# ChainSafe/halo2-verifier

Measured on NVIDIA B200. Metric: verified proofs/sec (BN254 SHPLONK, batch 4096), higher is better.
Workload: dtype u32x8 (256-bit Montgomery integers)

## Files before the change

__graft_entry__.py:

```python
import importlib.util
import os
import subprocess
import sys

ROOT = os.path.dirname(os.path.abspath(__file__))
PKG_DIR = os.path.join(ROOT, "halo2-verifier_b200")
CSRC = os.path.join(PKG_DIR, "csrc")
LIB = os.path.join(PKG_DIR, "libh2v_b200.so")
HOSTLIB = os.path.join(ROOT, "tests", "hostlib")
ORACLE = os.path.join(ROOT, "oracle")

NVCC_FLAGS = [
    "-gencode", "arch=compute_100a,code=sm_100a", "-lineinfo", "-O3", "-std=c++17",
    "-Xcompiler", "-fPIC", "-shared", "-I", os.path.join(ROOT, "include"), "-I", CSRC,
]


def load_package():
    name = "halo2_verifier_b200"
    if name in sys.modules:
        return sys.modules[name]
    spec = importlib.util.spec_from_file_location(name, os.path.join(PKG_DIR, "__init__.py"),
                                                  submodule_search_locations=[PKG_DIR])
    mod = importlib.util.module_from_spec(spec)
    sys.modules[name] = mod
    spec.loader.exec_module(mod)
    return mod


def _newer(target, sources):
    if not os.path.exists(target):
        return True
    t = os.path.getmtime(target)
    return any(os.path.getmtime(s) > t for s in sources)


def _run(cmd):
    print("+", " ".join(cmd), flush=True)
    subprocess.run(cmd, check=True)


def build(force=False):
    headers = [os.path.join(CSRC, f) for f in os.listdir(CSRC)] + [os.path.join(ROOT, "include", "h2v.h")]
    if force or _newer(LIB, headers):
        nvcc = os.environ.get("NVCC", "/usr/local/cuda/bin/nvcc")
        _run([nvcc] + NVCC_FLAGS + [os.path.join(CSRC, "kernels.cu"), os.path.join(CSRC, "plan_build.cpp"), "-o", LIB])
    for name, srcs in (("libprim.so", ["prim_harness.cpp"]), ("libstage.so", ["stage_harness.cpp", os.path.join(CSRC, "plan_build.cpp")]),
                       ("libmix.so", ["mix_harness.cpp"]), ("libacc.so", ["acc_harness.cpp"]),
                       ("libagg.so", ["agg_harness.cpp"])):
        out = os.path.join(HOSTLIB, name)
        full = [s if os.path.isabs(s) else os.path.join(HOSTLIB, s) for s in srcs]
        if force or _newer(out, headers + full):
            cmd = ["g++", "-O2", "-std=c++17", "-shared", "-fPIC", "-I", CSRC]
            for s in full:
                cmd += ["-x", "c++", s]
            _run(cmd + ["-o", out])
    mk = os.path.join(ORACLE, "Makefile")
    if os.path.exists(mk):
        _run(["make", "-s", "-C", ORACLE])
    load_package()


def smoke():
    import random

    sys.path.insert(0, ORACLE)
    import bn254 as bn
    import prover_sim as sim
    import verifier as orc

    pkg = load_package()
    rng = random.Random(11)
    k, s = 8, sim.FIXTURE_SRS_SECRET
    params = sim.make_params(k, s)
    vk, dl = sim.make_vk("vm", k)
    n = 8
    instances = [sim.random_instances(vk, rng, 10) for _ in range(n)]
    proofs = [sim.simulate_proof(params, vk, dl, s, inst, rng) for inst in instances]
    proofs[3], _ = sim.corrupt(proofs[3], vk, "eval_flip", rng)
    rs = [rng.randrange(1, bn.R) for _ in range(n)]
    bv = pkg.BatchVerifier(pkg.ParamsKZG.from_bytes(params.to_bytes()), pkg.VerifyingKey.from_bytes(vk.to_bytes(1)), device=0)
    res = bv.verify_batch(proofs, [i[0] for i in instances], rlc_scalars=rs, want_challenges=True, want_batch_accum=True)
    want = [orc.verify_proof(params, vk, inst, p) for inst, p in zip(instances, proofs)]
    assert res.status == [w.status for w in want], (res.status, [w.status for w in want])
    C = bv.n_challenges
    for j, w in enumerate(want):
        got = [int.from_bytes(res.challenges[32 * (j * C + c): 32 * (j * C + c + 1)], "little") for c in range(C)]
        assert got == w.challenges, f"challenge mismatch on proof {j}"
    L, Rr, _ok = orc.accumulate(params, want, rs)
    enc = lambda p: bytes(64) if p is None else p[0].to_bytes(32, "little") + p[1].to_bytes(32, "little")
    assert res.batch_accum == enc(L) + enc(Rr), "folded accumulator mismatch"
    print("smoke ok: statuses", res.status, "launches", bv.launch_count(), "timings(ms)", bv.timings())
    bv.close()


if __name__ == "__main__":
    build(force="--force" in sys.argv)
    if "--smoke" in sys.argv:
        smoke()
```

halo2-verifier_b200/csrc/kernels.cu:

```cuda
#include <cuda_runtime.h>
#include <nvtx3/nvToolsExt.h>
#include <errno.h>
#include <stdio.h>
#include <string.h>
#include <sys/random.h>
#include <time.h>
#include <unistd.h>

#include <algorithm>
#include <cmath>
#include <string>
#include <vector>

#include "h2v.h"
#include "plan_build.h"
#include "stages.cuh"
#include "tower.cuh"
#include "timeline.cuh"
#include "pairing_cta.cuh"
#include "exchange.cuh"
#include "transcript_quad.cuh"
#include "glv.cuh"
#include "mix.cuh"
#include "acc.cuh"
#include "agg.cuh"

using namespace h2v;

#ifndef H2V_TRANSCRIPT_MINB
#define H2V_TRANSCRIPT_MINB 1
#endif
#ifndef H2V_SCALAR_MINB
#define H2V_SCALAR_MINB 1
#endif

__device__ __forceinline__ void pdl_prologue() {
  asm volatile("griddepcontrol.wait;" ::: "memory");
  asm volatile("griddepcontrol.launch_dependents;" ::: "memory");
}

__global__ void k_init(PlanView pv, u32 n, const u64* inst_off, const u32* ncols, const u32* col_len, u32* status, u32* bad) {
  pdl_prologue();
  const u32 j = blockIdx.x * blockDim.x + threadIdx.x;
  if (j >= n) return;
  const PlanHeader& hd = pv.h();
  bad[j] = H2V_NO_BAD_ITEM;
  const u64 tot = inst_off[j + 1] - inst_off[j];
  u32 st = ST_OK;
  if (ncols && ncols[j] != hd.n_inst_cols) {
    st = ST_INVALID_INSTANCES;
  } else if (col_len) {
    u64 s = 0;
    for (u32 c = 0; c < hd.n_inst_cols; c++) s += col_len[(size_t)j * hd.n_inst_cols + c];
    if (s != tot) st = ST_INVALID_INSTANCES;
  } else if (hd.n_inst_cols == 0 ? tot != 0 : (tot % hd.n_inst_cols) != 0) {
    st = ST_INVALID_INSTANCES;
  }
  status[j] = st;
}

__global__ void __launch_bounds__(128) k_decompress(PlanView pv, u32 n, const u8* proofs, const u64* proof_off, G1Affine* pts, u32* ptsc, u32* bad, u32 blk_off, u32 blk_total) {
  pdl_prologue();
  TlScope tl_(1, pts);
  const PlanHeader& hd = pv.h();
  for (u32 t = (blk_off + blockIdx.x) * blockDim.x + threadIdx.x; t < n * hd.n_points; t += blk_total * blockDim.x) {
    const u32 j = t % n, slot = t / n;
    const u64 off = proof_off[j];
    const u32 len = (u32)(proof_off[j + 1] - off);
    G1Affine p;
    Fq canon[2];
    if (!decompress_stage(pv, proofs + off, len, slot, p, ptsc ? canon : nullptr)) {
      p.x = Fq::zero();
      p.y = Fq::zero();
      canon[0] = Fq::zero();
      canon[1] = Fq::zero();
      atomicMin(&bad[j], pv.sec<u32>(hd.off_pt_item)[slot]);
    }
    pts[t] = p;
    if (ptsc) {
      uint4* o = (uint4*)(ptsc + 16 * (size_t)t);
      o[0] = make_uint4(canon[0].l[0], canon[0].l[1], canon[0].l[2], canon[0].l[3]);
      o[1] = make_uint4(canon[0].l[4], canon[0].l[5], canon[0].l[6], canon[0].l[7]);
      o[2] = make_uint4(canon[1].l[0], canon[1].l[1], canon[1].l[2], canon[1].l[3]);
      o[3] = make_uint4(canon[1].l[4], canon[1].l[5], canon[1].l[6], canon[1].l[7]);
    }
  }
}

template <class H>
__global__ void __launch_bounds__(64, H2V_TRANSCRIPT_MINB) k_transcript(PlanView pv, u32 n, const u8* proofs, const u64* proof_off, const u8* inst,
                                                   const u64* inst_off, const G1Affine* pts, Fr* vals, u32* status, const u32* bad) {
  pdl_prologue();
  TlScope tl_(2, pts);
  const PlanHeader& hd = pv.h();
  for (u32 j = blockIdx.x * blockDim.x + threadIdx.x; j < n; j += gridDim.x * blockDim.x) {
    if (status[j] != ST_OK) continue;
    const u64 off = proof_off[j];
    bool inst_bad;
    const u32 b = transcript_stage<H>(pv, proofs + off, (u32)(proof_off[j + 1] - off), inst + 32 * inst_off[j],
                                      (u32)(inst_off[j + 1] - inst_off[j]), pts, vals, j, n, bad[j], inst_bad);
    if (inst_bad) status[j] = ST_INVALID_INSTANCES;
    else if (b != H2V_NO_BAD_ITEM) status[j] = b < hd.first_mo_item ? ST_TRANSCRIPT : ST_OPENING;
  }
}

__global__ void __launch_bounds__(4 * TQ_PROOFS_PER_BLOCK) k_transcript_quad(PlanView pv, u32 n, const u8* proofs, const u64* proof_off, const u8* inst, const u64* inst_off,
                                                                             const u32* ptsc, Fr* vals, u32* status, const u32* bad) {
  pdl_prologue();
// ... 319 lines not shown
    cnt[threadIdx.x * SCAN_PER + q] = 0;
  }
  u32 e = block_excl_scan<SCAN_NT>(sum, &total);
#pragma unroll
  for (u32 q = 0; q < SCAN_PER; q++) {
    base[threadIdx.x * SCAN_PER + q] = e;
    e += v[q];
  }
  __syncthreads();
  u32 bin[SCAN_PER], local[SCAN_PER];
#pragma unroll
  for (u32 q = 0; q < SCAN_PER; q++) {
    const u32 i = blockIdx.x * SCAN_TILE + q * SCAN_NT + threadIdx.x;
    if (i < nb) {
      bin[q] = size_bin(hist[i]);
      local[q] = atomicAdd(&cnt[bin[q]], 1u);
    }
  }
  __syncthreads();
#pragma unroll
  for (u32 q = 0; q < SCAN_PER; q++) {
    const u32 b = threadIdx.x * SCAN_PER + q;
    if (cnt[b]) cnt[b] = atomicAdd(&size_cursor[b], cnt[b]);
  }
  __syncthreads();
#pragma unroll
  for (u32 q = 0; q < SCAN_PER; q++) {
    const u32 i = blockIdx.x * SCAN_TILE + q * SCAN_NT + threadIdx.x;
    if (i < nb) order[base[bin[q]] + cnt[bin[q]] + local[q]] = i;
  }
}

template <class Src>
__global__ void __launch_bounds__(256) k_msm_scatter(MsmGeom g, const int16_t* dig, u32* cursor, u32* sorted, Src src) {
  pdl_prologue();
  TlScope tl_(5, sorted);
  const u64 total = ((u64)g.G * g.T << g.glv) * g.Wmax;
  for (u64 idx = (u64)blockIdx.x * blockDim.x + threadIdx.x; idx < total; idx += (u64)gridDim.x * blockDim.x) {
    const u32 row = (u32)(idx / g.Wmax), w = (u32)(idx % g.Wmax);
    const u32 t = row >> g.glv;
    u32 ch;
    if constexpr (Src::mixed) {
      const MixSeg& sg = src.seg[mix_segment(src.seg, src.count, t)];
      ch = mix_channel(mix_term(sg, t - sg.t0));
    } else {
      ch = g.channel_of_term(t % g.T);
    }
    if (w >= g.W[ch]) continue;
    const int d = dig[idx];
    if (d == 0) continue;
    const u32 b = (t / g.T) * g.nb() + g.bbase[ch] + w * g.B[ch] + (u32)(d < 0 ? -d : d) - 1;
    const u32 pos = atomicAdd(&cursor[b], 1u);
    sorted[pos] = row | (d < 0 ? 0x80000000u : 0u);
  }
}

__device__ __forceinline__ G1Jac shfl_down_jac(const G1Jac& p, u32 delta) {
  G1Jac r;
#pragma unroll
  for (int i = 0; i < 8; i++) {
    r.X.l[i] = __shfl_down_sync(0xFFFFFFFFu, p.X.l[i], delta);
    r.Y.l[i] = __shfl_down_sync(0xFFFFFFFFu, p.Y.l[i], delta);
    r.Z.l[i] = __shfl_down_sync(0xFFFFFFFFu, p.Z.l[i], delta);
  }
  return r;
}

#ifndef GLV_BUCKET_LANES
#define GLV_BUCKET_LANES 2
#endif
template <class Src>
__device__ __forceinline__ const G1Affine& term_point(const MsmGeom& g, u32 t, const G1Affine* pts, const G1Affine* shared_pts, const Src& src) {
  if constexpr (Src::mixed) {
    const MixSeg& sg = src.seg[mix_segment(src.seg, src.count, t)];
    return mix_point(sg, mix_term(sg, t - sg.t0));
  } else {
    return msm_point(g, t, pts, shared_pts);
  }
}
template <bool GLV, int LANES, class Src>
__global__ void __launch_bounds__(128) k_msm_bucket_sum(MsmGeom g, u32 nb, const u32* off, const u32* order, const u32* sorted,
                                                        const G1Affine* pts, const G1Affine* shared_pts, G1Jac* buckets, u32 blk_off, u32 blk_total,
                                                        Src src) {
  pdl_prologue();
  TlScope tl_(6, pts);
  if constexpr (LANES > 1) {
    for (u32 t0 = (blk_off + blockIdx.x) * blockDim.x; t0 < LANES * nb; t0 += blk_total * blockDim.x) {
      const u32 t = t0 + threadIdx.x, q = t % LANES;
      const bool live = t / LANES < nb;
      const u32 b = live ? order[t / LANES] : 0;
      G1Jac acc = G1Jac::identity();
      if (live) {
        const u32 e1 = off[b + 1];
        for (u32 e = off[b] + q; e < e1; e += LANES) {
          const u32 ent = sorted[e], row = ent & 0x7FFFFFFFu;
          if constexpr (GLV) {
            static_assert(!Src::mixed, "mixed batches have no GLV split");
            G1Affine pt = msm_point(g, row >> 1, pts, shared_pts);
            if (row & 1) pt.x = Fq::mul_c(pt.x, glv_beta());
            acc = g1_add_mixed(acc, pt, (ent >> 31) != 0);
          } else {
            acc = g1_add_mixed(acc, term_point(g, row, pts, shared_pts, src), (ent >> 31) != 0);
          }
        }
      }
#pragma unroll
      for (u32 d = LANES / 2; d >= 1; d >>= 1) acc = g1_add(acc, shfl_down_jac(acc, d));
      if (live && q == 0) buckets[b] = acc;
    }
  } else {
    static_assert(!GLV, "the GLV variant shares its buckets between lanes");
    for (u32 t = (blk_off + blockIdx.x) * blockDim.x + threadIdx.x; t < nb; t += blk_total * blockDim.x) {
      const u32 b = order[t];
      G1Jac acc = G1Jac::identity();
      const u32 e0 = off[b], e1 = off[b + 1];
      for (u32 e = e0; e < e1; e++) {
        const u32 ent = sorted[e];
        acc = g1_add_mixed(acc, term_point(g, ent & 0x7FFFFFFFu, pts, shared_pts, src), (ent >> 31) != 0);
      }
      buckets[b] = acc;
    }
  }
}

__device__ G1Jac g1_mul_small(const G1Jac& p, u32 k) {
  G1Jac acc = G1Jac::identity();
  if (k == 0) return acc;
  for (int i = 31 - __clz(k); i >= 0; i--) {
    acc = g1_double(acc);
    if ((k >> i) & 1) acc = g1_add(acc, p);
  }
  return acc;
}

__global__ void __launch_bounds__(128, 4) k_msm_chunk_reduce(MsmGeom g, u32 n_chunks, const G1Jac* buckets, G1Jac* partials) {
  pdl_prologue();
  TlScope tl_(7, buckets);
  for (u32 q = blockIdx.x * blockDim.x + threadIdx.x; q < n_chunks; q += gridDim.x * blockDim.x) {
    const u32 b0 = q * g.m, bl = b0 % g.nb();
    const u32 ch = bl >= g.bbase[1] ? 1u : 0u;
    const u32 i0 = (bl - g.bbase[ch]) % g.B[ch];
    G1Jac run = G1Jac::identity(), acc = G1Jac::identity();
    for (u32 i = g.m; i-- > 0;) {
      run = g1_add(run, buckets[b0 + i]);
      acc = g1_add(acc, run);
    }
    if (i0) acc = g1_add(acc, g1_mul_small(run, i0));
    partials[q] = acc;
  }
}

__global__ void __launch_bounds__(128) k_msm_window_reduce(MsmGeom g, const G1Jac* partials, G1Jac* window_sums) {
  pdl_prologue();
  TlScope tl_(8, window_sums);
  __shared__ G1Jac sh[128];
  const u32 Wt = g.W[0] + g.W[1];
  const u32 grp = blockIdx.x / Wt, wi = blockIdx.x % Wt, t = threadIdx.x;
  const u32 ch = wi >= g.wbase[1] ? 1u : 0u;
  const u32 per = g.B[ch] / g.m;
  const G1Jac* p = partials + (grp * g.nb() + g.bbase[ch] + (wi - g.wbase[ch]) * g.B[ch]) / g.m;
  G1Jac total = G1Jac::identity();
  for (u32 i = t; i < per; i += 128) total = g1_add(total, p[i]);
  sh[t] = total;
  __syncthreads();
  for (u32 d = 64; d > 0; d >>= 1) {
    if (t < d) sh[t] = g1_add(sh[t], sh[t + d]);
    __syncthreads();
  }
  if (t == 0) window_sums[blockIdx.x] = sh[0];
}

struct FoldArgs {
  u32 W[2], c[2], wbase[2];
};

__device__ __forceinline__ void store_affine_bytes(const G1Affine& a, bool is_id, u8* out) {
  if (is_id) {
    for (int i = 0; i < 64; i++) out[i] = 0;
    return;
  }
  a.x.to_canonical().store_le(out);
  a.y.to_canonical().store_le(out + 32);
}

__global__ void __launch_bounds__(32) k_fold_accum(FoldArgs fa, const G1Jac* window_sums, u8* acc_bytes) {
  pdl_prologue();
  const int t = threadIdx.x;
  if (t >= 2) return;
  G1Jac acc = G1Jac::identity();
  const G1Jac* wsum = window_sums + fa.wbase[t];
  for (u32 w = fa.W[t]; w-- > 0;) {
    for (u32 i = 0; i < fa.c[t]; i++) g1_double_inl(acc);
    acc = g1_add(acc, wsum[w]);
  }
  G1Affine a;
  const bool id = !g1_to_affine_inl(acc, a);
  store_affine_bytes(a, id, acc_bytes + 64 * (t == 0 ? 1 : 0));
}

struct GroupArgs {
  u32 W[2], c[2], wbase[2];
  u32 P[2], pbase[2];
  u32 run;
};
__global__ void __launch_bounds__(64) k_window_group(GroupArgs ga, u32 groups, const G1Jac* __restrict__ wsums, G1Jac* __restrict__ out) {
// ... 385 lines not shown
    cudaError_t e = cudaMallocHost(&p, want);
    if (e == cudaSuccess) cap = want;
    return e;
  }
  void release() {
    if (p) cudaFreeHost(p);
    p = nullptr;
    cap = 0;
  }
  template <class T>
  T* as() const {
    return (T*)p;
  }
};

struct h2v_ctx {
  int device = -1;
  cudaStream_t stream = nullptr;
  cudaStream_t stream_aux = nullptr;
  cudaEvent_t ev_fork = nullptr, ev_join = nullptr, ev_done = nullptr;
  bool blocking_sync = false;
  std::vector<u8> blob;
  PlanInfo info{};
  PlanHeader hd{};
  std::string err;
  u64 launches = 0;
  cudaEvent_t ev[8]{};
  float timings[8]{};
  const u32* opt_ncols = nullptr;
  const u32* opt_col_len = nullptr;
  u8* opt_scalar_hook = nullptr;
  u32 n = 0;
  u64 gbase = 0, gcount = 0;
  bool has_ncols = false, has_col_len = false;
  u32 scratch_rows = 0;
  MsmGeom geom{};
  bool ran = false;
  u32 opt_fold_groups = 0;
  std::vector<u32> h_verdicts;
  bool verdicts_on_device = false;
  u32 opt_shard_hint = 0;
  bool opt_has_key = false;
  RlcKey opt_key{};
  u32 rlc_source = 0;
  bool opt_has_agg_scalar = false;
  Fr opt_agg_scalar{}, h_rho{};
  struct LinesSlot {
    u64 key = ~0ull, used = 0;
    DevBuf buf;
  } lines[4];
  int lines_cur = -1;
  u64 lines_builds = 0;
  u64 use_clock = 0;
  bool use_graphs = true;
  bool use_pdl = false;
  bool capturing = false;
  bool stages_timed = false;
  struct GraphSlot {
    u64 key = 0, used = 0;
    u64 kernels = 0;
    cudaGraphExec_t exec = nullptr;
  } graphs[16];
  u64 graph_captures = 0;
  struct AbsorbTarget {
    G1Jac *acc = nullptr, *records = nullptr;
    u32* count = nullptr;
    u32 cap = 0;
  } absorb;
  struct Comm {
    bool ready = false;
    XLayout lay{};
    u8* window = nullptr;
    std::vector<u8*> peers;
    std::vector<void*> opened;
    u8** d_peers = nullptr;
    XDyn* d_dyn = nullptr;
    u32* d_done = nullptr;
    XDyn* h_dyn = nullptr;
    u32 ring = 0;
    u64 seq = 0;
    u64 timeout_ns = 30ull * 1000000000ull;
  } comm;
  struct MsmBufs {
    DevBuf coef, shared_sum, dig, hist, off, cursor, order, sorted, buckets, wsums, partials_msm, tiles;
  } mb, ab;
  DevBuf d_plan, d_proofs, d_proof_off, d_inst, d_inst_off, d_ncols, d_col_len, d_pts, d_bad, d_status, d_vals, d_scratch, d_right,
      d_shared, d_left, d_rlc_bytes, d_r, d_acc_bytes, d_verdict, d_partials, d_pp_prod, d_pp_lr, d_pp_bytes, d_hook, d_chal, d_flush, d_M, d_partial_out,
      d_wsums_fin, d_sub_pairs, d_sub_verdict, d_sub_M, d_gsums, d_ptsc, d_rho;
  const G2Line* d_lines() const { return lines_cur >= 0 ? lines[lines_cur].buf.as<G2Line>() : nullptr; }
  std::vector<DevBuf*> all_bufs() {
    std::vector<DevBuf*> v = {&d_plan, &d_proofs, &d_proof_off, &d_inst, &d_inst_off, &d_ncols, &d_col_len, &d_pts, &d_bad, &d_status, &d_vals, &d_scratch,
                              &d_right, &d_shared, &d_left, &d_rlc_bytes, &d_r, &d_acc_bytes, &d_verdict, &d_partials, &d_pp_prod, &d_pp_lr, &d_pp_bytes,
                              &d_hook, &d_chal, &d_flush, &d_M, &d_partial_out, &d_wsums_fin, &d_sub_pairs, &d_sub_verdict, &d_sub_M, &d_gsums, &d_ptsc, &d_rho,
                              &lines[0].buf, &lines[1].buf, &lines[2].buf, &lines[3].buf};
    for (MsmBufs* m : {&mb, &ab})
      for (DevBuf* d : {&m->coef, &m->shared_sum, &m->dig, &m->hist, &m->off, &m->cursor, &m->order, &m->sorted, &m->buckets, &m->wsums, &m->partials_msm, &m->tiles})
        v.push_back(d);
    return v;
  }
  HostBuf h_status, h_verd;
  PlanView pv() const { return PlanView{d_plan.as<u8>()}; }
};

#define CKC(call)                                                                  \
  do {                                                                             \
    cudaError_t e_ = (call);                                                       \
    if (e_ != cudaSuccess) {                                                       \
      ctx->err = std::string(#call) + ": " + cudaGetErrorString(e_);               \
      return -2;                                                                   \
    }                                                                              \
  } while (0)
#define LAUNCH_CHECK()                       \
  do {                                       \
    ctx->launches++;                         \
    CKC(cudaGetLastError());                 \
  } while (0)

static inline u32 cdiv(u64 a, u32 b) { return (u32)((a + b - 1) / b); }

struct NvtxRange {
  explicit NvtxRange(const char* name) { nvtxRangePushA(name); }
  ~NvtxRange() { nvtxRangePop(); }
};

static bool trace_on() {
  static const bool on = getenv("H2V_TRACE") != nullptr;
  return on;
}
static void trace(const h2v_ctx* ctx, const char* what) {
  if (!trace_on()) return;
  timespec ts;
  clock_gettime(CLOCK_MONOTONIC, &ts);
  fprintf(stderr, "[h2v %p %ld.%06ld] %s\n", (const void*)ctx, (long)(ts.tv_sec % 1000), ts.tv_nsec / 1000, what);
}

static u32 wide_grid(u64 items, u32 dflt_per_sm) {
  static const int sms = [] {
    int dev = 0, n = 148;
    cudaGetDevice(&dev);
    cudaDeviceGetAttribute(&n, cudaDevAttrMultiProcessorCount, dev);
    return n;
  }();
  static const int env = getenv("H2V_WIDE_BLOCKS_PER_SM") ? atoi(getenv("H2V_WIDE_BLOCKS_PER_SM")) : -1;
  const u32 per_sm = env >= 0 ? (u32)env : dflt_per_sm;
  const u32 full = cdiv(items, 128);
  return per_sm ? std::min<u32>(full, (u32)sms * per_sm) : full;
}

static u32 wide_split() {
  static const u32 k = [] {
    const char* e = getenv("H2V_WIDE_SPLIT");
    const int v = e ? atoi(e) : 1;
    return (u32)(v >= 1 && v <= 64 ? v : 1);
  }();
  return k;
}

static u32 narrow_grid(u64 units) {
  static const u32 cap = [] {
    const char* e = getenv("H2V_NARROW_BLOCKS_PER_SM");
    const int v = e ? atoi(e) : 0;
    return (u32)(v > 0 ? v * 148 : 0);
  }();
  const u32 u = (u32)std::min<u64>(units, 0x7FFFFFFFu);
  return cap ? std::min(u, cap) : u;
}

// ... 210 lines not shown

static int launch_pairing(h2v_ctx* ctx, const MsmGeom& g, const G2Line* lines, const G1Jac* wsums, u32 groups) {
  const MsmGeom q = pair_geom(g, groups);
  cudaStream_t s = ctx->stream;
  const PairSkip none{nullptr, nullptr, 1, 0};
  const u32 np = q.W[0] + q.W[1];
  const G1Jac* pairs = wsums;
  if (line_run(groups) > 1) {
    GroupArgs ga{{g.W[0], g.W[1]}, {g.c[0], g.c[1]}, {0, g.W[0]}, {q.W[0], q.W[1]}, {0, q.W[0]}, line_run(groups)};
    KLAUNCH(k_window_group, cdiv((u64)groups * np, 64), 64, 0, s, ga, groups, wsums, ctx->d_gsums.as<G1Jac>());
    pairs = ctx->d_gsums.as<G1Jac>();
  }
  KLAUNCH((k_lines<LINES_GROUPS>), dim3(H2V_ATE_ITERS, groups), 64 * LINES_GROUPS, k_lines_smem<LINES_GROUPS>(), s, LinesArgs{np}, pairs, lines,
                                                                                       ctx->d_M.as<E12>(), none);
  static const bool seg_off = getenv("H2V_MILLER_SEGMENTS_OFF") != nullptr;
  if (groups * MILLER_SEGS <= 148 && !seg_off) {
    E12* seg = ctx->d_M.as<E12>() + (size_t)groups * H2V_ATE_ITERS;
    KLAUNCH(k_miller_segments, dim3(MILLER_SEGS, groups), 128, 0, s, ctx->d_M.as<E12>(), seg);
    KLAUNCH(k_pairing_check<true>, groups, 128, 0, s, seg, ctx->d_verdict.as<u32>(), none);
  } else {
    KLAUNCH(k_pairing_check<false>, groups, 128, 0, s, ctx->d_M.as<E12>(), ctx->d_verdict.as<u32>(), none);
  }
  return 0;
}
static int launch_pairing(h2v_ctx* ctx, const G1Jac* wsums, u32 groups) { return launch_pairing(ctx, ctx->geom, ctx->d_lines(), wsums, groups); }

static int launch_pair_checks(h2v_ctx* ctx, const G1Jac* pairs, u32 count, const G2Line* unit_lines, E12* M, u32* verdict, PairSkip sk) {
  cudaStream_t s = ctx->stream;
  KLAUNCH_P(false, (k_lines<2>), dim3(H2V_ATE_ITERS, count), 128, k_lines_smem<2>(), s, LinesArgs{2}, pairs, unit_lines, M, sk);
  KLAUNCH_P(false, k_pairing_check<false>, count, 128, 0, s, M, verdict, sk);
  return 0;
}

static int read_verdicts(h2v_ctx* ctx, u32* all, bool xchg = false) {
  const u32 G = ctx->geom.G ? ctx->geom.G : 1;
  CKC(ctx->h_verd.ensure(4 * (size_t)(G + 2)));
  u32* hv = ctx->h_verd.as<u32>();
  hv[G] = hv[G + 1] = 0;
  CKC(cudaMemcpyAsync(hv, ctx->d_verdict.p, 4 * (size_t)(G + (xchg ? 2 : 0)), cudaMemcpyDeviceToHost, ctx->stream));
  CKC(ctx_sync(ctx));
  ctx->h_verdicts.assign(hv, hv + G + 2);
  const u32 e_local = ctx->h_verdicts[G], e_root = ctx->h_verdicts[G + 1];
  ctx->h_verdicts.resize(G);
  if (xchg && ((e_local | e_root) & 5)) {
    ctx->err = std::string("sharded exchange timed out: ") +
               ((e_local & 1) ? "this rank is the root and a peer's partial accumulators never arrived"
                : (e_root & 1) ? "the root reports that a peer's partial accumulators never arrived"
                               : "the root's verdicts never arrived") +
               " (a rank died, or the ranks disagree on the launch-set order of this channel)";
    return -3;
  }
  if (xchg && ((e_local | e_root) & 2)) {
    ctx->err = "partial accumulators were produced with different window geometries (use h2v_batch_set_shard_hint)";
    return -1;
  }
  u32 a = 1;
  for (u32 v : ctx->h_verdicts) a &= v ? 1u : 0u;
  *all = a;
  return 0;
}

static cudaError_t preload_kernels() {
  cudaFuncAttributes fa;
  cudaError_t e = cudaSuccess;
#define H2V_PRELOAD(k) \
  if (e == cudaSuccess) e = cudaFuncGetAttributes(&fa, k)
  H2V_PRELOAD(k_init);
  H2V_PRELOAD(k_decompress);
  H2V_PRELOAD(k_transcript<Blake2b>);
  H2V_PRELOAD(k_transcript<Keccak256>);
  H2V_PRELOAD(k_transcript_quad);
  H2V_PRELOAD(k_scalar<H2V_SCALAR_MINB>);
  H2V_PRELOAD(k_scalar<12>);
  H2V_PRELOAD(k_rlc_expand);
  H2V_PRELOAD(k_rlc_scan);
  H2V_PRELOAD(k_shared_reduce);
  H2V_PRELOAD(k_msm_digits<SingleVkTerms>);
  H2V_PRELOAD(k_msm_digits<MixTerms>);
  H2V_PRELOAD(k_scan_tiles);
  H2V_PRELOAD(k_scan_apply);
  H2V_PRELOAD(k_bucket_order);
  H2V_PRELOAD(k_msm_scatter<SingleVkTerms>);
  H2V_PRELOAD(k_msm_scatter<MixTerms>);
  H2V_PRELOAD((k_msm_bucket_sum<false, 1, SingleVkTerms>));
  H2V_PRELOAD((k_msm_bucket_sum<false, 2, SingleVkTerms>));
  H2V_PRELOAD((k_msm_bucket_sum<false, 4, SingleVkTerms>));
  H2V_PRELOAD((k_msm_bucket_sum<true, GLV_BUCKET_LANES, SingleVkTerms>));
  H2V_PRELOAD((k_msm_bucket_sum<false, 1, MixTerms>));
  H2V_PRELOAD((k_msm_bucket_sum<false, 2, MixTerms>));
  H2V_PRELOAD((k_msm_bucket_sum<false, 4, MixTerms>));
  H2V_PRELOAD(k_msm_chunk_reduce);
  H2V_PRELOAD(k_msm_window_reduce);
  H2V_PRELOAD(k_fold_accum);
  H2V_PRELOAD(k_window_group);
  H2V_PRELOAD(k_pack_partial);
  H2V_PRELOAD(k_sum_partials);
  H2V_PRELOAD(k_pp_mul);
  H2V_PRELOAD(k_pp_reduce);
  H2V_PRELOAD(k_window_combine);
  H2V_PRELOAD(k_pp_suspects);
  H2V_PRELOAD(k_pp_mul_list);
  H2V_PRELOAD(k_pp_reduce_list);
  H2V_PRELOAD(k_pp_status);
  H2V_PRELOAD(k_acc_absorb);
  H2V_PRELOAD(k_agg);
  H2V_PRELOAD(k_lines<2>);
  H2V_PRELOAD(k_gather_scalars);
  H2V_PRELOAD(k_gather_challenges);
  H2V_PRELOAD(k_lines<LINES_GROUPS>);
  H2V_PRELOAD(k_pairing_check<false>);
  H2V_PRELOAD(k_pairing_check<true>);
  H2V_PRELOAD(k_miller_segments);
  H2V_PRELOAD(k_pack_partial_x);
  H2V_PRELOAD(k_bcast_verdict);
  H2V_PRELOAD(k_wait_verdict);
#undef H2V_PRELOAD
  return e;
}

struct CommHandle {
  u32 magic, rank, world, max_groups;
  u64 pid, ptr, bytes;
  int device, rsv;
  cudaIpcMemHandle_t ipc;
  u8 pad[H2V_COMM_HANDLE_BYTES - 48 - sizeof(cudaIpcMemHandle_t)];
};
static_assert(sizeof(CommHandle) == H2V_COMM_HANDLE_BYTES, "comm handle size");
static constexpr u32 H2V_COMM_MAGIC = 0x58563248u;
static constexpr u32 XDYN_RING = 64;

static void comm_release(h2v_ctx* ctx) {
  h2v_ctx::Comm& cm = ctx->comm;
  for (void* p : cm.opened) cudaIpcCloseMemHandle(p);
  cm.opened.clear();
  cm.peers.clear();
  if (cm.window) cudaFree(cm.window);
  if (cm.d_peers) cudaFree(cm.d_peers);
  if (cm.d_dyn) cudaFree(cm.d_dyn);
  if (cm.d_done) cudaFree(cm.d_done);
  if (cm.h_dyn) cudaFreeHost(cm.h_dyn);
  cm = h2v_ctx::Comm{};
}

extern "C" {

const char* h2v_last_error(const h2v_ctx* ctx) { return ctx ? ctx->err.c_str() : g_create_error.c_str(); }

int h2v_ctx_create(h2v_ctx** out, const uint8_t* params, size_t params_len, int params_format, const uint8_t* vk, size_t vk_len,
                   int vk_format, int multiopen, int hash, int device) {
  return h2v_ctx_create_multi(out, params, params_len, params_format, vk, vk_len, vk_format, multiopen, hash, device, 1);
}

}

static int ctx_create(h2v_ctx** out, const uint8_t* params, size_t params_len, int params_format, const uint8_t* vk, size_t vk_len, int vk_format,
                      int multiopen, int hash, int device, uint32_t circuit_instances, const AggSpec* agg) {
  if (!out || !params || !vk) {
    g_create_error = "null argument";
    return -1;
  }
  h2v_ctx* ctx = new h2v_ctx();
  std::string err;
  if (build_plan(params, params_len, params_format, vk, vk_len, vk_format, multiopen, hash, ctx->blob, ctx->info, err, circuit_instances, agg) != 0) {
    g_create_error = err;
    h2v_ctx_destroy(ctx);
    return -1;
  }
  memcpy(&ctx->hd, ctx->blob.data(), sizeof(PlanHeader));
  int count = 0;
  cudaError_t e = cudaGetDeviceCount(&count);
  if (e != cudaSuccess || device < 0 || device >= count) {
// ... 173 lines not shown
      const u32 m = S.pt_end - S.pt_begin;
      mm += si == 0 ? m : (S.diff_end - S.diff_begin) + 1;
      mm += (m - 1) + (double)m * m + 1 + 1;
      for (u32 c = S.cm_begin; c < S.cm_end; c++) mm += m + 3 + (sc[c].kind == CM_HMSM ? hd.n_h : 0);
    }
  } else {
    const GwcPoint* gp = pv.sec<GwcPoint>(hd.off_gwcpts);
    const GwcQuery* gq = pv.sec<GwcQuery>(hd.off_gwcq);
    for (u32 p = 0; p < hd.n_gwc_points; p++) {
      mm += 4;
      for (u32 q = gp[p].q_begin; q < gp[p].q_end; q++) mm += 3 + (gq[q].kind == CM_HMSM ? hd.n_h : 0);
    }
  }
  return mm;
}

extern "C" int h2v_ctx_work_model(const h2v_ctx* ctx, uint32_t instance_rows, double* out4) {
  if (!ctx || !out4) return -1;
  const PlanHeader& hd = ctx->hd;
  out4[0] = scalar_stage_mm(ctx->blob, instance_rows);
  out4[1] = 2.0 * hd.n_points + hd.n_scalars + 2.0 * hd.n_challenges;
  out4[2] = 250 + 38 + 16 + 9;
  out4[3] = (double)hd.n_inst_cols * instance_rows;
  return 0;
}

int h2v_ctx_vk_lint(const h2v_ctx* ctx, char* report, size_t capacity) {
  if (!ctx) return -1;
  std::string all;
  for (const std::string& f : ctx->info.lint) all += f + "\n";
  if (report && capacity) {
    const size_t k = std::min(capacity - 1, all.size());
    memcpy(report, all.data(), k);
    report[k] = 0;
  }
  return (int)ctx->info.lint.size();
}

int h2v_batch_set_columns(h2v_ctx* ctx, const uint32_t* inst_ncols, const uint32_t* inst_col_len) {
  if (!ctx) return -1;
  ctx->opt_ncols = inst_ncols;
  ctx->opt_col_len = inst_col_len;
  return 0;
}
int h2v_batch_set_fold_groups(h2v_ctx* ctx, uint32_t groups) {
  if (!ctx) return -1;
  ctx->opt_fold_groups = groups;
  return 0;
}
int h2v_last_group_verdicts(const h2v_ctx* ctx, uint8_t* out, uint32_t capacity) {
  if (!ctx || !ctx->ran) return -1;
  const u32 G = (u32)ctx->h_verdicts.size();
  for (u32 i = 0; i < G && i < capacity; i++) out[i] = ctx->h_verdicts[i] ? 1 : 0;
  return (int)G;
}

int h2v_batch_set_rlc_key(h2v_ctx* ctx, const uint8_t* key32) {
  if (!ctx || !key32) return -1;
  memcpy(ctx->opt_key.w, key32, 32);
  ctx->opt_has_key = true;
  return 0;
}
int h2v_last_rlc_source(const h2v_ctx* ctx) { return ctx ? (int)ctx->rlc_source : -1; }

int h2v_batch_set_shard_hint(h2v_ctx* ctx, uint32_t max_shard_proofs) {
  if (!ctx) return -1;
  ctx->opt_shard_hint = max_shard_proofs;
  return 0;
}
size_t h2v_partial_bytes(void) { return H2V_PARTIAL_BYTES; }
int h2v_batch_set_scalar_hook(h2v_ctx* ctx, uint8_t* msm_scalars) {
  if (!ctx) return -1;
  ctx->opt_scalar_hook = msm_scalars;
  return 0;
}

static int enqueue_shared_reduce(h2v_ctx* ctx, const MsmGeom& g, h2v_ctx::MsmBufs& B, cudaStream_t s) {
  const PlanHeader& hd = ctx->hd;
  if (hd.n_shared)
    KLAUNCH(k_shared_reduce, dim3(hd.n_shared, g.G), 256, 0, s, g.n, g.N, (u32)hd.n_shared, ctx->d_shared.as<Fr>(), B.coef.as<Fr>(), B.shared_sum.as<Fr>());
  return 0;
}

struct TermArrays {
  const Fr *right, *left, *coef, *shared_sum;
  const G1Affine *pts, *shared_pts;
};

extern "C++" {
template <class Src>
static int enqueue_buckets(h2v_ctx* ctx, const MsmGeom& g, h2v_ctx::MsmBufs& B, cudaStream_t s, const TermArrays& ta, Src src,
                           const u32* parent_verdict, u32 parent_size) {
  const u32 nb = g.nb() * g.G;
  KLAUNCH(k_msm_digits<Src>, cdiv((u64)g.G * g.T, 128), 128, 0, s, g, ta.right, ta.left, ta.coef, ta.shared_sum, ta.shared_pts, B.dig.as<int16_t>(),
          B.hist.as<u32>(), parent_verdict, parent_size, src);
  const u32 n_tiles = cdiv(nb, SCAN_TILE);
  KLAUNCH(k_scan_tiles, n_tiles, SCAN_NT, 0, s, B.hist.as<u32>(), nb, B.off.as<u32>(), B.tiles.as<u32>(), B.hist.as<u32>() + nb);
  KLAUNCH(k_scan_apply, n_tiles, SCAN_NT, 0, s, nb, n_tiles, B.tiles.as<u32>(), B.off.as<u32>(), B.cursor.as<u32>());
  KLAUNCH(k_bucket_order, n_tiles, SCAN_NT, 0, s, nb, B.hist.as<u32>(), B.hist.as<u32>() + nb, B.hist.as<u32>() + nb + SIZE_BINS, B.order.as<u32>());
  KLAUNCH(k_msm_scatter<Src>, std::min<u32>(cdiv(((u64)g.G * g.T << g.glv) * g.Wmax, 256), 148 * 16), 256, 0, s, g, B.dig.as<int16_t>(), B.cursor.as<u32>(),
          B.sorted.as<u32>(), src);
  {
    set_launch_class('W');
    static const int lanes_env = getenv("H2V_BUCKET_LANES") ? atoi(getenv("H2V_BUCKET_LANES")) : 0;
    const u32 lanes = g.glv ? GLV_BUCKET_LANES : (lanes_env ? (u32)lanes_env : (g.G == 1 && g.n <= 8192 ? 2u : 1u));
    void (*kern)(MsmGeom, u32, const u32*, const u32*, const u32*, const G1Affine*, const G1Affine*, G1Jac*, u32, u32, Src);
    kern = lanes == 2 ? k_msm_bucket_sum<false, 2, Src> : lanes == 4 ? k_msm_bucket_sum<false, 4, Src> : k_msm_bucket_sum<false, 1, Src>;
    if constexpr (!Src::mixed)
      if (g.glv) kern = k_msm_bucket_sum<true, GLV_BUCKET_LANES, Src>;
    const u32 total = wide_grid((u64)(lanes == 2 || lanes == 4 || g.glv ? lanes : 1u) * nb, 0), K = std::min(wide_split(), total), per = cdiv(total, K);
    for (u32 off = 0; off < total; off += per)
      KLAUNCH(kern, std::min(per, total - off), 128, 0, s, g, nb, B.off.as<u32>(), B.order.as<u32>(), B.sorted.as<u32>(), ta.pts, ta.shared_pts,
              B.buckets.as<G1Jac>(), off, total, src);
  }
  set_launch_class('N');
  if (g.B[0] == g.m && g.B[1] == g.m) {
    KLAUNCH(k_msm_chunk_reduce, narrow_grid(cdiv(nb / g.m, 128)), 128, 0, s, g, nb / g.m, B.buckets.as<G1Jac>(), B.wsums.as<G1Jac>());
  } else {
    KLAUNCH(k_msm_chunk_reduce, narrow_grid(cdiv(nb / g.m, 128)), 128, 0, s, g, nb / g.m, B.buckets.as<G1Jac>(), B.partials_msm.as<G1Jac>());
    KLAUNCH(k_msm_window_reduce, (g.W[0] + g.W[1]) * g.G, 128, 0, s, g, B.partials_msm.as<G1Jac>(), B.wsums.as<G1Jac>());
  }
  return 0;
}
}

static int enqueue_msm(h2v_ctx* ctx, const MsmGeom& g, h2v_ctx::MsmBufs& B, cudaStream_t s, const u32* parent_verdict, u32 parent_size) {
  int rc = enqueue_shared_reduce(ctx, g, B, s);
  if (rc) return rc;
  PlanView pv = ctx->pv();
  const TermArrays ta{ctx->d_right.as<Fr>(), ctx->d_left.as<Fr>(), B.coef.as<Fr>(), B.shared_sum.as<Fr>(), ctx->d_pts.as<G1Affine>(),
                      pv.sec<G1Affine>(ctx->hd.off_shared_pts)};
  return enqueue_buckets(ctx, g, B, s, ta, SingleVkTerms{}, parent_verdict, parent_size);
}

static cudaError_t ensure_msm_bufs(const MsmGeom& g, h2v_ctx::MsmBufs& B, u32 n_shared) {
  const size_t nb = (size_t)g.nb() * g.G;
  cudaError_t e;
  if ((e = B.coef.ensure(32 * (size_t)g.N)) != cudaSuccess) return e;
  if ((e = B.shared_sum.ensure(32 * (size_t)n_shared * g.G + 32)) != cudaSuccess) return e;
  if ((e = B.dig.ensure(2 * ((size_t)g.G * g.T << g.glv) * g.Wmax)) != cudaSuccess) return e;
  if ((e = B.hist.ensure(4 * (nb + 2 * SIZE_BINS))) != cudaSuccess) return e;
  if ((e = B.order.ensure(4 * nb)) != cudaSuccess) return e;
  if ((e = B.off.ensure(4 * (nb + 1))) != cudaSuccess) return e;
  if ((e = B.cursor.ensure(4 * nb)) != cudaSuccess) return e;
  if ((e = B.tiles.ensure(4 * (nb / 1024 + 2))) != cudaSuccess) return e;
  if ((e = B.sorted.ensure(4 * ((size_t)g.G * g.T << g.glv) * g.Wmax)) != cudaSuccess) return e;
  if ((e = B.buckets.ensure(sizeof(G1Jac) * nb)) != cudaSuccess) return e;
  if ((e = B.wsums.ensure(sizeof(G1Jac) * (size_t)(g.W[0] + g.W[1]) * g.G)) != cudaSuccess) return e;
  return B.partials_msm.ensure(sizeof(G1Jac) * (nb / g.m));
}

static int upload_impl(h2v_ctx* ctx, u32 n, const u8* proofs, const u64* proof_off, const u8* instances, const u64* inst_off,
                       const u8* rlc, u64 seed, u64 gbase, u64 gcount) {
  if (!ctx) return -1;
  NvtxRange nv_("h2v:upload");
  ctx->ran = false;
  const u32 groups = ctx->opt_fold_groups ? ctx->opt_fold_groups : 1;
  ctx->opt_fold_groups = 0;
  if (n == 0 || !proof_off || !inst_off || (!proofs && proof_off[n]) || groups > 1024 || n % groups != 0 || gcount < gbase + n / groups) {
    ctx->err = "bad batch arguments (with fold groups the batch must split into equal groups)";
    return -1;
  }
  if (rlc && !fold_scalars_ok(rlc, gcount * groups)) {
    ctx->err = FOLD_SCALARS_ERR;
    return -1;
  }
  CKC(cudaSetDevice(ctx->device));
  const PlanHeader& hd = ctx->hd;
  const size_t pbytes = proof_off[n] - proof_off[0], iscal = inst_off[n] - inst_off[0];
  if (proof_off[0] != 0 || inst_off[0] != 0 || (iscal && !instances)) {
    ctx->err = "offset arrays must start at 0";
    return -1;
  }
  for (u32 j = 0; j < n; j++) {
    if (proof_off[j + 1] < proof_off[j] || inst_off[j + 1] < inst_off[j] || proof_off[j + 1] - proof_off[j] > 0x7FFFFFFFull ||
        inst_off[j + 1] - inst_off[j] > 0x03FFFFFFull) {
      ctx->err = "offset arrays must be non-decreasing with per-proof sizes below 2^31 bytes / 2^26 scalars";
      return -1;
    }
  }
  {
    const u64 terms = (u64)n * (msm_points(hd) + msm_mo(hd)) + (u64)hd.n_shared * groups;
    const u64 widest = std::max<u64>(std::max<u64>(msm_points(hd), hd.n_vals), msm_points(hd) + hd.n_shared + msm_mo(hd));
    if (terms >= (1ull << 31) || (u64)n * widest >= (1ull << 32)) {
      ctx->err = "batch too large for the 32-bit index space of the MSM (split it into several uploads)";
      return -1;
    }
  }
  u32 max_len = 0;
  if (ctx->opt_col_len) {
    for (size_t i = 0; i < (size_t)n * hd.n_inst_cols; i++) max_len = std::max(max_len, ctx->opt_col_len[i]);
  } else if (hd.n_inst_cols) {
    for (u32 j = 0; j < n; j++) max_len = std::max<u32>(max_len, (u32)((inst_off[j + 1] - inst_off[j]) / hd.n_inst_cols));
  }
  ctx->scratch_rows = hd.inst_max_rot + max_len + hd.inst_min_rot_abs + 1;
  if ((u64)n * ctx->scratch_rows * 32 > (16ull << 30)) {
    ctx->err = "instance columns too long for this batch size (Lagrange scratch would exceed 16 GiB)";
    return -1;
  }
  ctx->n = n;
  ctx->gbase = gbase;
  ctx->gcount = gcount;
  ctx->verdicts_on_device = false;
  ctx->geom = choose_geom(n / groups, hd, ctx->opt_shard_hint, groups);
  ctx->opt_shard_hint = 0;
  const MsmGeom& g = ctx->geom;
  const u32 nb = g.nb() * g.G;
  {
    int lrc = ensure_lines(ctx, groups);
    if (lrc) return lrc;
  }
  trace(ctx, "lines ready");
  CKC(ctx->d_proofs.ensure(pbytes + 64));
  CKC(ctx->d_proof_off.ensure(8 * (size_t)(n + 1)));
  CKC(ctx->d_inst.ensure(32 * iscal + 64));
  CKC(ctx->d_inst_off.ensure(8 * (size_t)(n + 1)));
  CKC(ctx->d_pts.ensure(sizeof(G1Affine) * (size_t)n * msm_points(hd)));
  if (hd.hash == HASH_BLAKE2B) CKC(ctx->d_ptsc.ensure(64 * (size_t)n * hd.n_points));
  CKC(ctx->d_bad.ensure(4 * (size_t)n));
  CKC(ctx->d_status.ensure(4 * (size_t)n));
  CKC(ctx->d_vals.ensure(32 * (size_t)n * hd.n_vals));
  CKC(ctx->d_scratch.ensure(32 * (size_t)n * ctx->scratch_rows));
  CKC(ctx->d_right.ensure(32 * (size_t)n * msm_points(hd)));
  CKC(ctx->d_shared.ensure(32 * (size_t)n * hd.n_shared));
  CKC(ctx->d_left.ensure(32 * (size_t)n * msm_mo(hd)));
  CKC(ctx->d_r.ensure(32 * (size_t)gcount * groups));
  CKC(ctx->d_partial_out.ensure((size_t)H2V_PARTIAL_BYTES * groups));
  CKC(ctx->d_wsums_fin.ensure(sizeof(G1Jac) * 128 * (size_t)groups));
  CKC(ctx->d_gsums.ensure(sizeof(G1Jac) * 128 * (size_t)groups));
  CKC(ensure_msm_bufs(g, ctx->mb, hd.n_shared));
// ... 1583 lines not shown
```

Baseline: 6.746 million.

## Sum single-lane MSM buckets with batched-inversion affine pairwise additions

Replaces the one-lane-per-bucket Jacobian accumulation kernel with an affine bucket reduction. Each thread processes its strided buckets over several levels of pairwise affine additions, sharing one field inversion per level through a Montgomery batch-inversion prefix product, then finishes the remaining points with mixed Jacobian adds. This cuts the field multiplications per point addition, but adds a serial inversion per level, scratch buffers in global memory for points and prefix products, and extra memory traffic. The level count comes from an environment variable and defaults to 2, and the grid size now uses occupancy.

```diff
diff --git a/__graft_entry__.py b/__graft_entry__.py
--- a/__graft_entry__.py
+++ b/__graft_entry__.py
@@ -47,7 +47,7 @@
         _run([nvcc] + NVCC_FLAGS + [os.path.join(CSRC, "kernels.cu"), os.path.join(CSRC, "plan_build.cpp"), "-o", LIB])
     for name, srcs in (("libprim.so", ["prim_harness.cpp"]), ("libstage.so", ["stage_harness.cpp", os.path.join(CSRC, "plan_build.cpp")]),
                        ("libmix.so", ["mix_harness.cpp"]), ("libacc.so", ["acc_harness.cpp"]),
-                       ("libagg.so", ["agg_harness.cpp"])):
+                       ("libagg.so", ["agg_harness.cpp"]), ("libbucket.so", ["bucket_harness.cpp"])):
         out = os.path.join(HOSTLIB, name)
         full = [s if os.path.isabs(s) else os.path.join(HOSTLIB, s) for s in srcs]
         if force or _newer(out, headers + full):
diff --git a/halo2-verifier_b200/csrc/bucket_affine.cuh b/halo2-verifier_b200/csrc/bucket_affine.cuh
--- /dev/null
+++ b/halo2-verifier_b200/csrc/bucket_affine.cuh
@@ -0,0 +1,93 @@
+#pragma once
+#include "curve.cuh"
+
+namespace h2v {
+
+H2V_HD bool aff_is_identity(const G1Affine& p) { return p.x.is_zero(); }
+
+H2V_HD Fq pair_denom(const G1Affine& p, const G1Affine& q) {
+  if (aff_is_identity(p) || aff_is_identity(q)) return Fq::one();
+  if (p.x != q.x) return q.x - p.x;
+  return p.y == q.y ? p.y.dbl() : Fq::one();
+}
+
+H2V_HD G1Affine pair_sum(const G1Affine& p, const G1Affine& q, const Fq& inv) {
+  if (aff_is_identity(p)) return q;
+  if (aff_is_identity(q)) return p;
+  Fq lam;
+  if (p.x != q.x) {
+    lam = (q.y - p.y) * inv;
+  } else if (p.y == q.y) {
+    const Fq xx = p.x.sqr();
+    lam = (xx.dbl() + xx) * inv;
+  } else {
+    return G1Affine{Fq::zero(), Fq::zero()};
+  }
+  G1Affine r;
+  r.x = lam.sqr() - p.x - q.x;
+  r.y = lam * (p.x - r.x) - p.y;
+  return r;
+}
+
+template <class Src0>
+struct BucketLane {
+  const u32 *order, *off;
+  u32 k0, stride, nq;
+  Src0 src;
+  G1Affine* scr;
+  Fq* pf;
+
+  H2V_HD u32 bucket(u32 j) const { return order[k0 + stride * j]; }
+  H2V_HD u32 base(u32 b) const { return off[b] / 2 + b; }
+  H2V_HD u32 count(u32 b, u32 lv) const {
+    const u32 m = off[b + 1] - off[b];
+    return m == 0 ? 0u : ((m - 1) >> lv) + 1;
+  }
+  H2V_HD Fq x(u32 b, u32 lv, u32 i) const { return lv == 0 ? src.x(off[b] + i) : scr[base(b) + i].x; }
+  H2V_HD G1Affine pt(u32 b, u32 lv, u32 i) const { return lv == 0 ? src.pt(off[b] + i) : scr[base(b) + i]; }
+
+  H2V_HD void level(u32 lv) const {
+    Fq acc = Fq::one();
+    bool any = false;
+    for (u32 j = nq; j-- > 0;) {
+      const u32 b = bucket(j), np = count(b, lv) / 2, s = base(b);
+      for (u32 i = np; i-- > 0;) {
+        const Fq x1 = x(b, lv, 2 * i), x2 = x(b, lv, 2 * i + 1);
+        Fq d;
+        if (x1.is_zero() || x2.is_zero()) d = Fq::one();
+        else if (x1 != x2) d = x2 - x1;
+        else d = pair_denom(pt(b, lv, 2 * i), pt(b, lv, 2 * i + 1));
+        pf[s + i] = acc;
+        acc = acc * d;
+        any = true;
+      }
+    }
+    Fq inv = any ? acc.inv_bin() : acc;
+    for (u32 j = 0; j < nq; j++) {
+      const u32 b = bucket(j), n = count(b, lv), np = n / 2, s = base(b);
+      for (u32 i = 0; i < np; i++) {
+        const G1Affine p = pt(b, lv, 2 * i), q = pt(b, lv, 2 * i + 1);
+        const Fq ik = inv * pf[s + i];
+        inv = inv * pair_denom(p, q);
+        scr[s + i] = pair_sum(p, q, ik);
+      }
+      if (n & 1) scr[s + np] = pt(b, lv, n - 1);
+    }
+  }
+
+  template <class Out>
+  H2V_HD void run(u32 L, Out out) const {
+    for (u32 lv = 0; lv < L; lv++) level(lv);
+    for (u32 j = 0; j < nq; j++) {
+      const u32 b = bucket(j), n = count(b, L), s = base(b);
+      G1Jac acc = G1Jac::identity();
+      for (u32 i = 0; i < n; i++) {
+        const G1Affine p = scr[s + i];
+        if (!aff_is_identity(p)) acc = g1_add_mixed(acc, p);
+      }
+      out(b, acc);
+    }
+  }
+};
+
+}
diff --git a/halo2-verifier_b200/csrc/kernels.cu b/halo2-verifier_b200/csrc/kernels.cu
--- a/halo2-verifier_b200/csrc/kernels.cu
+++ b/halo2-verifier_b200/csrc/kernels.cu
@@ -24,6 +24,7 @@
 #include "mix.cuh"
 #include "acc.cuh"
 #include "agg.cuh"
+#include "bucket_affine.cuh"
 
 using namespace h2v;
 
@@ -509,45 +510,59 @@
 __global__ void __launch_bounds__(128) k_msm_bucket_sum(MsmGeom g, u32 nb, const u32* off, const u32* order, const u32* sorted,
                                                         const G1Affine* pts, const G1Affine* shared_pts, G1Jac* buckets, u32 blk_off, u32 blk_total,
                                                         Src src) {
+  static_assert(LANES > 1, "one lane per bucket is k_msm_bucket_affine");
   pdl_prologue();
   TlScope tl_(6, pts);
-  if constexpr (LANES > 1) {
-    for (u32 t0 = (blk_off + blockIdx.x) * blockDim.x; t0 < LANES * nb; t0 += blk_total * blockDim.x) {
-      const u32 t = t0 + threadIdx.x, q = t % LANES;
-      const bool live = t / LANES < nb;
-      const u32 b = live ? order[t / LANES] : 0;
-      G1Jac acc = G1Jac::identity();
-      if (live) {
-        const u32 e1 = off[b + 1];
-        for (u32 e = off[b] + q; e < e1; e += LANES) {
-          const u32 ent = sorted[e], row = ent & 0x7FFFFFFFu;
-          if constexpr (GLV) {
-            static_assert(!Src::mixed, "mixed batches have no GLV split");
-            G1Affine pt = msm_point(g, row >> 1, pts, shared_pts);
-            if (row & 1) pt.x = Fq::mul_c(pt.x, glv_beta());
-            acc = g1_add_mixed(acc, pt, (ent >> 31) != 0);
-          } else {
-            acc = g1_add_mixed(acc, term_point(g, row, pts, shared_pts, src), (ent >> 31) != 0);
-          }
+  for (u32 t0 = (blk_off + blockIdx.x) * blockDim.x; t0 < LANES * nb; t0 += blk_total * blockDim.x) {
+    const u32 t = t0 + threadIdx.x, q = t % LANES;
+    const bool live = t / LANES < nb;
+    const u32 b = live ? order[t / LANES] : 0;
+    G1Jac acc = G1Jac::identity();
+    if (live) {
+      const u32 e1 = off[b + 1];
+      for (u32 e = off[b] + q; e < e1; e += LANES) {
+        const u32 ent = sorted[e], row = ent & 0x7FFFFFFFu;
+        if constexpr (GLV) {
+          static_assert(!Src::mixed, "mixed batches have no GLV split");
+          G1Affine pt = msm_point(g, row >> 1, pts, shared_pts);
+          if (row & 1) pt.x = Fq::mul_c(pt.x, glv_beta());
+          acc = g1_add_mixed(acc, pt, (ent >> 31) != 0);
+        } else {
+          acc = g1_add_mixed(acc, term_point(g, row, pts, shared_pts, src), (ent >> 31) != 0);
         }
       }
+    }
 #pragma unroll
-      for (u32 d = LANES / 2; d >= 1; d >>= 1) acc = g1_add(acc, shfl_down_jac(acc, d));
-      if (live && q == 0) buckets[b] = acc;
-    }
-  } else {
-    static_assert(!GLV, "the GLV variant shares its buckets between lanes");
-    for (u32 t = (blk_off + blockIdx.x) * blockDim.x + threadIdx.x; t < nb; t += blk_total * blockDim.x) {
-      const u32 b = order[t];
-      G1Jac acc = G1Jac::identity();
-      const u32 e0 = off[b], e1 = off[b + 1];
-      for (u32 e = e0; e < e1; e++) {
-        const u32 ent = sorted[e];
-        acc = g1_add_mixed(acc, term_point(g, ent & 0x7FFFFFFFu, pts, shared_pts, src), (ent >> 31) != 0);
-      }
-      buckets[b] = acc;
-    }
-  }
+    for (u32 d = LANES / 2; d >= 1; d >>= 1) acc = g1_add(acc, shfl_down_jac(acc, d));
+    if (live && q == 0) buckets[b] = acc;
+  }
+}
+
+template <class Src>
+struct SortedTermPoints {
+  const MsmGeom& g;
+  const u32* sorted;
+  const G1Affine *pts, *shared_pts;
+  const Src& src;
+  __device__ __forceinline__ Fq x(u32 e) const { return term_point(g, sorted[e] & 0x7FFFFFFFu, pts, shared_pts, src).x; }
+  __device__ __forceinline__ G1Affine pt(u32 e) const {
+    const u32 ent = sorted[e];
+    G1Affine p = term_point(g, ent & 0x7FFFFFFFu, pts, shared_pts, src);
+    if (ent >> 31) p.y = p.y.neg();
+    return p;
+  }
+};
+
+template <class Src>
+__global__ void __launch_bounds__(128) k_msm_bucket_affine(MsmGeom g, u32 nb, u32 L, const u32* off, const u32* order, const u32* sorted,
+                                                           const G1Affine* pts, const G1Affine* shared_pts, G1Affine* scr, Fq* pf, G1Jac* buckets,
+                                                           u32 blk_off, u32 blk_total, Src src) {
+  pdl_prologue();
+  TlScope tl_(6, pts);
+  const u32 t = (blk_off + blockIdx.x) * blockDim.x + threadIdx.x, T = blk_total * blockDim.x;
+  const u32 nq = t < nb ? (nb - t + T - 1) / T : 0u;
+  const BucketLane<SortedTermPoints<Src>> lane{order, off, t, T, nq, SortedTermPoints<Src>{g, sorted, pts, shared_pts, src}, scr, pf};
+  lane.run(L, [&](u32 b, const G1Jac& acc) { buckets[b] = acc; });
 }
 
 __device__ G1Jac g1_mul_small(const G1Jac& p, u32 k) {
@@ -1099,7 +1114,7 @@
     u64 timeout_ns = 30ull * 1000000000ull;
   } comm;
   struct MsmBufs {
-    DevBuf coef, shared_sum, dig, hist, off, cursor, order, sorted, buckets, wsums, partials_msm, tiles;
+    DevBuf coef, shared_sum, dig, hist, off, cursor, order, sorted, buckets, wsums, partials_msm, tiles, aff_pts, aff_pf;
   } mb, ab;
   DevBuf d_plan, d_proofs, d_proof_off, d_inst, d_inst_off, d_ncols, d_col_len, d_pts, d_bad, d_status, d_vals, d_scratch, d_right,
       d_shared, d_left, d_rlc_bytes, d_r, d_acc_bytes, d_verdict, d_partials, d_pp_prod, d_pp_lr, d_pp_bytes, d_hook, d_chal, d_flush, d_M, d_partial_out,
@@ -1476,11 +1491,11 @@
   H2V_PRELOAD(k_bucket_order);
   H2V_PRELOAD(k_msm_scatter<SingleVkTerms>);
   H2V_PRELOAD(k_msm_scatter<MixTerms>);
-  H2V_PRELOAD((k_msm_bucket_sum<false, 1, SingleVkTerms>));
+  H2V_PRELOAD(k_msm_bucket_affine<SingleVkTerms>);
   H2V_PRELOAD((k_msm_bucket_sum<false, 2, SingleVkTerms>));
   H2V_PRELOAD((k_msm_bucket_sum<false, 4, SingleVkTerms>));
   H2V_PRELOAD((k_msm_bucket_sum<true, GLV_BUCKET_LANES, SingleVkTerms>));
-  H2V_PRELOAD((k_msm_bucket_sum<false, 1, MixTerms>));
+  H2V_PRELOAD(k_msm_bucket_affine<MixTerms>);
   H2V_PRELOAD((k_msm_bucket_sum<false, 2, MixTerms>));
   H2V_PRELOAD((k_msm_bucket_sum<false, 4, MixTerms>));
   H2V_PRELOAD(k_msm_chunk_reduce);
@@ -1820,12 +1835,29 @@
   return 0;
 }
 
+static u32 bucket_affine_levels() {
+  static const u32 l = [] {
+    const char* e = getenv("H2V_BUCKET_AFFINE_LEVELS");
+    const int v = e ? atoi(e) : 0;
+    return (u32)(v >= 1 && v <= 16 ? v : 2);
+  }();
+  return l;
+}
 struct TermArrays {
   const Fr *right, *left, *coef, *shared_sum;
   const G1Affine *pts, *shared_pts;
 };
 
 extern "C++" {
+template <class Src>
+static u32 bucket_affine_blocks_per_sm() {
+  static const u32 n = [] {
+    int b = 0;
+    if (cudaOccupancyMaxActiveBlocksPerMultiprocessor(&b, k_msm_bucket_affine<Src>, 128, 0) != cudaSuccess || b < 1) b = 1;
+    return (u32)b;
+  }();
+  return n;
+}
 template <class Src>
 static int enqueue_buckets(h2v_ctx* ctx, const MsmGeom& g, h2v_ctx::MsmBufs& B, cudaStream_t s, const TermArrays& ta, Src src,
                            const u32* parent_verdict, u32 parent_size) {
@@ -1842,14 +1874,21 @@
     set_launch_class('W');
     static const int lanes_env = getenv("H2V_BUCKET_LANES") ? atoi(getenv("H2V_BUCKET_LANES")) : 0;
     const u32 lanes = g.glv ? GLV_BUCKET_LANES : (lanes_env ? (u32)lanes_env : (g.G == 1 && g.n <= 8192 ? 2u : 1u));
-    void (*kern)(MsmGeom, u32, const u32*, const u32*, const u32*, const G1Affine*, const G1Affine*, G1Jac*, u32, u32, Src);
-    kern = lanes == 2 ? k_msm_bucket_sum<false, 2, Src> : lanes == 4 ? k_msm_bucket_sum<false, 4, Src> : k_msm_bucket_sum<false, 1, Src>;
-    if constexpr (!Src::mixed)
-      if (g.glv) kern = k_msm_bucket_sum<true, GLV_BUCKET_LANES, Src>;
-    const u32 total = wide_grid((u64)(lanes == 2 || lanes == 4 || g.glv ? lanes : 1u) * nb, 0), K = std::min(wide_split(), total), per = cdiv(total, K);
-    for (u32 off = 0; off < total; off += per)
-      KLAUNCH(kern, std::min(per, total - off), 128, 0, s, g, nb, B.off.as<u32>(), B.order.as<u32>(), B.sorted.as<u32>(), ta.pts, ta.shared_pts,
-              B.buckets.as<G1Jac>(), off, total, src);
+    if (lanes == 1 && !g.glv) {
+      const u32 total = wide_grid(nb, bucket_affine_blocks_per_sm<Src>()), K = std::min(wide_split(), total), per = cdiv(total, K);
+      for (u32 off = 0; off < total; off += per)
+        KLAUNCH(k_msm_bucket_affine<Src>, std::min(per, total - off), 128, 0, s, g, nb, bucket_affine_levels(), B.off.as<u32>(), B.order.as<u32>(),
+                B.sorted.as<u32>(), ta.pts, ta.shared_pts, B.aff_pts.as<G1Affine>(), B.aff_pf.as<Fq>(), B.buckets.as<G1Jac>(), off, total, src);
+    } else {
+      void (*kern)(MsmGeom, u32, const u32*, const u32*, const u32*, const G1Affine*, const G1Affine*, G1Jac*, u32, u32, Src);
+      kern = lanes == 4 ? k_msm_bucket_sum<false, 4, Src> : k_msm_bucket_sum<false, 2, Src>;
+      if constexpr (!Src::mixed)
+        if (g.glv) kern = k_msm_bucket_sum<true, GLV_BUCKET_LANES, Src>;
+      const u32 total = wide_grid((u64)lanes * nb, 0), K = std::min(wide_split(), total), per = cdiv(total, K);
+      for (u32 off = 0; off < total; off += per)
+        KLAUNCH(kern, std::min(per, total - off), 128, 0, s, g, nb, B.off.as<u32>(), B.order.as<u32>(), B.sorted.as<u32>(), ta.pts, ta.shared_pts,
+                B.buckets.as<G1Jac>(), off, total, src);
+    }
   }
   set_launch_class('N');
   if (g.B[0] == g.m && g.B[1] == g.m) {
@@ -1884,6 +1923,11 @@
   if ((e = B.tiles.ensure(4 * (nb / 1024 + 2))) != cudaSuccess) return e;
   if ((e = B.sorted.ensure(4 * ((size_t)g.G * g.T << g.glv) * g.Wmax)) != cudaSuccess) return e;
   if ((e = B.buckets.ensure(sizeof(G1Jac) * nb)) != cudaSuccess) return e;
+  if (!g.glv) {
+    const size_t slots = ((size_t)g.G * g.T * g.Wmax) / 2 + nb;
+    if ((e = B.aff_pts.ensure(sizeof(G1Affine) * slots)) != cudaSuccess) return e;
+    if ((e = B.aff_pf.ensure(sizeof(Fq) * slots)) != cudaSuccess) return e;
+  }
   if ((e = B.wsums.ensure(sizeof(G1Jac) * (size_t)(g.W[0] + g.W[1]) * g.G)) != cudaSuccess) return e;
   return B.partials_msm.ensure(sizeof(G1Jac) * (nb / g.m));
 }
```

After: 7.025 million, median of 6. +4.1%, better.
